# smoggy-P/gym-Drone2D-ActivePerception

Hardware: AMD Instinct MI355X
Metric: env-steps/sec (batched) at 10 agents, map_id=1 (higher is better)
Workload: dtype f64

## Files before the change

gym-drone2d-activeperception_amd/csrc/d2d_hip.hip:

```cpp
#include <hip/hip_runtime.h>
#include <math.h>
#include <stdint.h>
#include <stdio.h>
#include <stdlib.h>
#include <string.h>
#include <type_traits>

#if defined(__HIP_DEVICE_COMPILE__)
#define D2D_AS __attribute__((address_space(1)))
#endif
#include "../../include/d2d.h"
#include "../../include/d2d_hooks.h"
#include "../../include/d2d_stepped.h"
#include "../../include/d2d_swept.h"

#define D2D_TAN_QUAL __device__ __forceinline__
#define D2D_TAN_TBL_QUAL __device__ const
#include "d2d_tan.h"
#define D2D_LOG_QUAL __device__ __forceinline__
#define D2D_LOG_TBL_QUAL __device__ const
#define D2D_RNG_QUAL __device__ __forceinline__
#include "d2d_rng.h"

#define WAVE 64
// ... 647 lines not shown
  }
  return ncand;
}

template <typename M>
struct RayT {
  double xs, ys;
  M cmask;
};
template <typename M>
__device__ __forceinline__ int mask_first(M m) {
  if constexpr (sizeof(M) == 8) return __ffsll((long long)m) - 1;
  else return __ffs((int)m) - 1;
}

template <typename M>
__device__ __forceinline__ RayT<M> ray_setup(const d2d_cfg &c, const LdsView &L, int i, int ncand, double x0, double y0,
                                             double yaw0) {
  const double ss = c.scale - 1.0;
  const double rad90 = 0x1.921fb54442d18p+0, rad270 = 0x1.2d97c7f3321d2p+2;
  const double pi_ = 0x1.921fb54442d18p+1;
  const double player_angle = 0x1.921fb54442d18p+2 - yaw0 * 0x1.1df46a2529d39p-6;
  const double ang = positive_angle(player_angle + (c.ray_off0 + c.ray_dth * (double)i));
  const bool faced_right = (ang < rad90 || ang > rad270);
  const bool faced_up = (ang > pi_);
#ifdef D2D_ABL_NOTAN
  double slope = ang * 0.3;
#else
  double slope = d2d_tan(ang);
#endif
  RayT<M> ry;
  if (fabs(slope) > 1.0) {
    slope = 1.0 / slope;
    ry.ys = faced_up ? -ss : ss;
    ry.xs = ry.ys * slope;
  } else {
    ry.xs = faced_right ? ss : -ss;
    ry.ys = ry.xs * slope;
  }
  ry.cmask = 0;
  if (ncand <= (int)(8 * sizeof(M))) {
    const double len2 = ry.xs * ry.xs + ry.ys * ry.ys, l1 = fabs(ry.xs) + fabs(ry.ys);
    for (int q = 0; q < ncand; ++q) {
      const double ex = L.cx[q] - x0, ey = L.cy[q] - y0, rq = L.crr[q] + 1e-6;
      const double cr = ex * ry.ys - ey * ry.xs, dt = ex * ry.xs + ey * ry.ys;
      const bool near_line = cr * cr <= rq * rq * len2 * (1.0 + 1e-9);
      const bool ahead = dt + rq * l1 >= 0.0;
      ry.cmask |= (near_line && ahead) ? (M)((M)1 << q) : (M)0;
    }
  }
  return ry;
}

template <bool GENERAL, bool FULL, typename M, typename GX>
__device__ __forceinline__ void ray_march(const GX &gx, const d2d_cfg &c, const Geom &g, const LdsView &L, const RayT<M> &ry, bool active,
                                          int ncand, double x0, double y0, const Tile &wt, const Tile &ct, bool patch,
                                          unsigned char *__restrict__ dm) {
  const int H = c.H;
  const CellDiv cell(c.scale, fmax(c.W_px, c.H_px));
  const double depth2 = c.depth * c.depth;
  const bool mask_path = ncand <= (int)(8 * sizeof(M));
  const unsigned char *gtw = (const unsigned char *)L.gtw;
  unsigned char *dmt = (unsigned char *)L.dmt;
  double x = x0 + ry.xs, y = y0 + ry.ys;
  bool alive = active && (0.0 < x && x < c.W_px && 0.0 < y && y < c.H_px);
  const int klo = g.klo;
  const bool has1 = mask_path && ry.cmask != (M)0;
  const int q1 = has1 ? mask_first(ry.cmask) : 0;
  const double c1x = L.cx[q1], c1y = L.cy[q1], c1r2 = has1 ? L.cr2[q1] : -1.0;
  const int c1i = L.cidx[q1];
  const M rest = mask_path ? (M)(ry.cmask & (ry.cmask - (M)1)) : (M)0;
  const bool some1 = __any(has1);
  auto sample = [&](auto far_tag) {
    constexpr bool FAR = decltype(far_tag)::value;
    bool any = false;
    if (some1) {
      const double dx = c1x - x, dy = c1y - y;
      any = alive && (dx * dx + dy * dy <= c1r2);
      if (any) L.hit[c1i] = 1;
    }
    if (GENERAL && mask_path) {
      M m = alive ? rest : (M)0;
      while (m) {
        const int q = mask_first(m);
        m &= m - (M)1;
        const double dx = L.cx[q] - x, dy = L.cy[q] - y;
        if (dx * dx + dy * dy <= L.cr2[q]) {
          L.hit[L.cidx[q]] = 1;
          any = true;
        }
      }
    } else if (GENERAL && alive) {
      if (ncand <= g.ccap) {
        for (int q = 0; q < ncand; ++q) {
          const double dx = L.cx[q] - x, dy = L.cy[q] - y;
          if (dx * dx + dy * dy <= L.cr2[q]) {
            L.hit[L.cidx[q]] = 1;
            any = true;
          }
        }
      } else {
        for (int k = 0; k < c.N; ++k) {
          const double dx = L.ax[k] - x, dy = L.ay[k] - y;
          if (dx * dx + dy * dy <= L.ar2[k]) {
            L.hit[k] = 1;
            any = true;
          }
        }
      }
    }
    const int ci = cell(x), cj = cell(y);
    unsigned int gi = 0;
    unsigned char wall;
    if constexpr (FULL) {
      gi = alive ? (unsigned int)(ci * H + cj) : 0u;
      wall = gtw[gi];
    } else {
      const int wr = min(max(ci - wt.i0, 0), wt.rows - 1), wq = min(max(cj - wt.j0, 0), wt.cols - 1);
      wall = gtw[wt.byte_index(wr, wq)];
    }
    bool far = false;
    if (FAR) far = ((x - x0) * (x - x0) + (y - y0) * (y - y0) >= depth2);
    const bool stop = (wall == D2D_OCCUPIED) || far;
    const bool write = alive && !any && (!stop || wall == D2D_OCCUPIED);
    if (write) {
      const unsigned char v = stop ? (unsigned char)D2D_OCCUPIED : (unsigned char)D2D_UNOCCUPIED;
      if constexpr (FULL) {
        dm[gi] = v;
        if (patch) dmt[gi] = v;
      } else {
        dm[(unsigned int)gx(ci, cj)] = v;
        const unsigned int pr = (unsigned int)(ci - ct.i0), pq = (unsigned int)(cj - ct.j0);
        if (patch && pr < (unsigned int)ct.rows && pq < (unsigned int)ct.cols) dmt[pr * ct.cols + pq] = v;
      }
    }
    alive = alive && !any && !stop;
    x = x + ry.xs;
    y = y + ry.ys;
    alive = alive && (0.0 < x && x < c.W_px && 0.0 < y && y < c.H_px);
  };
#ifndef D2D_ABL_NOMARCH
  const int k1 = min(klo + 1, g.smax);
#pragma unroll 1
  for (int k = 1; k < k1; ++k) sample(std::false_type{});
#pragma unroll 1
  for (int k = max(k1, 1); k < g.smax; ++k) sample(std::true_type{});
#endif
}

struct DynCells {
  unsigned int pclr;
  unsigned int nfree;
};

__device__ __forceinline__ void dyn_bitmap(const d2d_cfg &c, int lane, const Geom &g, const LdsView &L) {
  const int N = c.N, W = c.W, H = c.H;
  if (g.bmw == 0) return;
  for (int w = lane; w < g.bmw; w += WAVE) L.bm[w] = 0u;
  wave_sync_lds();
  for (int k = lane; k < N; k += WAVE) {
    const int cx = L.ncx[k], cy = L.ncy[k], u = L.nu[k];
    const int i1 = min(cx + u + 1, W), j1 = min(cy + u + 1, H);
    for (int i = max(cx - u, 0); i < i1; ++i)
      for (int j = max(cy - u, 0); j < j1; ++j) {
        const int bit = i * H + j;
        atomicOr(&L.bm[bit >> 5], 1u << (bit & 31));
      }
  }
}
// ... 662 lines not shown
    frz = ((double)r.steps >= c.max_steps && !dead) ? 1 : 0;
  }
  const int done = (col != 0) || dead || frz || (r.sm == D2D_SM_GOAL_REACHED && r.tnext >= r.ntgt);
  if (done && c.kf_enabled) {
    int an = 0, ats = 0;
    for (int k = lane; k < N; k += WAVE) {
      if (L.act[k] != 0) {
        an += 1;
        ats += L.klen[k];
      }
    }
    r.bufn += wave_sum(an);
    r.bufts += wave_sum(ats);
  }
  if (lane == 0) {
    unsigned char *f = s.flags + (size_t)e * 4;
    f[D2D_F_COLLISION] = (unsigned char)col;
    f[D2D_F_DEADLOCK] = (unsigned char)dead;
    f[D2D_F_FREEZING] = (unsigned char)frz;
    f[D2D_F_DONE] = (unsigned char)done;
  }
  r.done = done;
}

__device__ __forceinline__ void st_obs(const d2d_cfg &c, const d2d_state &s, int e, int lane, const LdsView &L,
                                       const EnvRegs &r) {
  const int n = c.L * c.L;
  unsigned char *__restrict__ ob = s.obs_local + (size_t)e * n;
  const unsigned char *dmt = (const unsigned char *)L.dmt;
  for (int idx = lane; idx < n; idx += WAVE) ob[idx] = dmt[idx];
  if (lane == 0) s.obs_yaw[e] = (float)r.yaw;
}

__device__ __forceinline__ void load_regs(const d2d_state &s, int e, EnvRegs &r) {
  const double *d = s.drone + (size_t)e * D2D_DF;
  r.x = d[D2D_D_X]; r.y = d[D2D_D_Y]; r.yaw = d[D2D_D_YAW];
  r.vx = d[D2D_D_VX]; r.vy = d[D2D_D_VY]; r.ax = d[D2D_D_AX]; r.ay = d[D2D_D_AY];
  r.tx = s.target[(size_t)e * 2]; r.ty = s.target[(size_t)e * 2 + 1];
  const int *cn = s.counters + (size_t)e * D2D_CF;
  r.steps = cn[D2D_C_STEPS]; r.fail = cn[D2D_C_FAIL]; r.sm = cn[D2D_C_SM]; r.tnext = cn[D2D_C_TGT_NEXT];
  r.ntgt = cn[D2D_C_NTGT]; r.tracked = cn[D2D_C_TRACKED]; r.bufn = cn[D2D_C_BUF_N]; r.bufts = cn[D2D_C_BUF_TS];
}

__device__ __forceinline__ void store_regs(const d2d_state &s, int e, const EnvRegs &r) {
  double *d = s.drone + (size_t)e * D2D_DF;
  d[D2D_D_X] = r.x; d[D2D_D_Y] = r.y; d[D2D_D_YAW] = r.yaw;
  d[D2D_D_VX] = r.vx; d[D2D_D_VY] = r.vy; d[D2D_D_AX] = r.ax; d[D2D_D_AY] = r.ay;
  s.target[(size_t)e * 2] = r.tx; s.target[(size_t)e * 2 + 1] = r.ty;
  int *cn = s.counters + (size_t)e * D2D_CF;
  cn[D2D_C_STEPS] = r.steps; cn[D2D_C_FAIL] = r.fail; cn[D2D_C_SM] = r.sm; cn[D2D_C_TGT_NEXT] = r.tnext;
  cn[D2D_C_TRACKED] = r.tracked; cn[D2D_C_BUF_N] = r.bufn; cn[D2D_C_BUF_TS] = r.bufts;
}

template <bool FULL, bool WIDE, bool CONE, bool TILED = false>
__device__ __forceinline__ void run_env(const d2d_cfg &c, const d2d_state &s, int e, int lane, uint32_t stages,
                                        const Geom &g, const LdsView &L, double action, EnvRegs &r, size_t noise_off = 0,
                                        bool load_r = false, const StepIn *given = nullptr, bool late_obs = false,
                                        int *dyn_gate = nullptr, bool dyn_visible = true, bool dyn_skip = false) {
  using RayMask = std::conditional_t<WIDE, unsigned long long, unsigned int>;
  const int N = c.N, W = c.W, H = c.H;
  const double inv_scale = 1.0 / c.scale;
  const bool do_ray = stages & D2D_ST_RAYCAST, do_dyn = (stages & D2D_ST_DYNGRID) && !dyn_skip, do_trk = stages & D2D_ST_TRACKER;
  const bool do_col = stages & D2D_ST_COLLIDE, do_obs = stages & D2D_ST_OBS, do_ctl = stages & D2D_ST_CONTROL;
  const GridIx<TILED> gx = {H, (H + 15) >> 4};
  const size_t gbytes = TILED ? (size_t)((W + 15) >> 4) * (size_t)((H + 15) >> 4) * 256 : (size_t)W * H;
  unsigned char *__restrict__ gt = s.gt + (size_t)e * gbytes;
  unsigned char *__restrict__ dm = s.dmap + (size_t)e * gbytes;

  const bool gt_staged = FULL && (do_ray || do_dyn);
  const uint32_t needs_agents = D2D_ST_AGENTS | D2D_ST_RAYCAST | D2D_ST_DYNGRID | D2D_ST_TRACKER | D2D_ST_COLLIDE;
  const bool agents_light = (stages & needs_agents) && !(stages & (D2D_ST_AGENTS | D2D_ST_RAYCAST | D2D_ST_DYNGRID));
  StepInRaw in_raw;
  AgentIn ag0;
  const bool agents_any = (stages & needs_agents) != 0;
  if (load_r) {
    in_raw.use = false;
    if (do_ctl && !given) load_inputs_raw(c, s, e, true, in_raw);
    agent_load(c, s, e, lane, do_trk || do_col, ag0, agents_light);
  }
  if constexpr (FULL) {
    if (gt_staged) grid_stage(gt, L.gtw, W * H, lane);
    if (do_obs) grid_stage(dm, L.dmt, W * H, lane);
  }
  if (load_r) {
    if (do_trk && c.kf_enabled && g.kf_lds) kf_stage(c, s, e, lane, L);
    load_regs(s, e, r);
    __builtin_amdgcn_sched_barrier(0);
  }
  StepIn in;
  if (given) {
    in = *given;
    in.action = action;
  } else if (load_r) {
    finish_inputs(in_raw, action, in);
  } else {
    load_inputs(c, s, e, action, do_ctl, in);
  }
  D2D_STAMP(1);
  if (stages & D2D_ST_FSM) st_fsm(c, s, e, r);
  const double x0 = r.x, y0 = r.y, yaw0 = r.yaw;
  if (do_ctl) st_control(c, in, r);
  D2D_STAMP(2);
  if (!load_r && do_trk && c.kf_enabled && g.kf_lds) kf_stage(c, s, e, lane, L);
  if (agents_any) {
    const bool move = (stages & D2D_ST_AGENTS) != 0;
    if (load_r) {
      if (lane < N) agent_apply(c, s, e, lane, L, inv_scale, move, agents_light, ag0);
      if (N > WAVE) st_agents(c, s, e, lane, g, L, inv_scale, move, do_trk || do_col, agents_light, WAVE);
    } else {
      st_agents_plain(c, s, e, lane, g, L, inv_scale, move, do_trk || do_col, agents_light, do_dyn || !dyn_gate);
    }
    if (do_trk && !do_ray)
      for (int k = lane; k < N; k += WAVE) L.hit[k] = s.hit[(size_t)e * N + k];
    wave_sync_lds();
  }
  D2D_STAMP(3);

  const int ocx = cell_fast(x0, c.scale, inv_scale), ocy = cell_fast(y0, c.scale, inv_scale);
  const int ncx_d = cell_fast(r.x, c.scale, inv_scale), ncy_d = cell_fast(r.y, c.scale, inv_scale);
  const int edge = (c.L - 1) / 2;
  const Tile wt = make_tile(ocx - g.reach, ocy - g.reach, g.ws, g.ws);
  const Tile ct = make_tile(ncx_d - edge, ncy_d - edge, c.L, c.L);
  bool probe_wall = false;
  const bool dyn_fast = do_dyn;
  DynCells dc;
  dc.pclr = dc.nfree = 0;
  if (do_col && lane < 5 && !gt_staged) {
    const double R = c.drone_radius;
    const double ox = (lane == 0) ? -R : (lane == 2 ? R : 0.0);
    const double oy = (lane == 3) ? -R : (lane == 4 ? R : 0.0);
    const double qx = r.x + ox, qy = r.y + oy;
    const bool oob = (qx >= c.W_px || qx < 0.0 || qy >= c.H_px || qy < 0.0);
    const int pi = min(max(cell_fast(qx, c.scale, inv_scale), 0), W - 1), pj = min(max(cell_fast(qy, c.scale, inv_scale), 0), H - 1);
    probe_wall = oob || gt[gx(pi, pj)] == D2D_OCCUPIED;
  }
  if constexpr (!FULL) {
    if (do_ray && do_obs && wt.cols <= 32 && wt.rows <= 24 && ct.cols <= 33 && ct.rows <= 34) {
      tile_rows2(gx, wt, (unsigned char *)L.gtw, gt, W, H, lane, (unsigned char)D2D_OCCUPIED,
                 ct, (unsigned char *)L.dmt, dm, (unsigned char)0);
    } else {
      if (do_ray) tile_load<9>(gx, wt, (unsigned char *)L.gtw, gt, W, H, lane, (unsigned char)D2D_OCCUPIED);
      if (do_obs) tile_load<9>(gx, ct, (unsigned char *)L.dmt, dm, W, H, lane, (unsigned char)0);
    }
    if (do_dyn) dyn_bitmap(c, lane, g, L);
    if (dyn_fast && lane < N) {
      if (g.dyn2p) dyn_load<true, false>(gx, c, gt, lane, L, dc);
      else dyn_load(gx, c, gt, lane, L, dc);
    }
  }

  int ncand = 0;
  if (do_ray) {
    ncand = ray_cull<CONE>(c, lane, L, x0, y0, yaw0, g.ccap);
  }
  wave_sync_lds();
  D2D_STAMP(4);
  auto landed = [&]() {
    asm volatile("s_waitcnt vmcnt(0)" ::: "memory");
    wave_sync_lds();
    if constexpr (FULL) {
      if (do_col && lane < 5 && gt_staged) {
        const double R = c.drone_radius;
        const double ox = (lane == 0) ? -R : (lane == 2 ? R : 0.0);
        const double oy = (lane == 3) ? -R : (lane == 4 ? R : 0.0);
        const double qx = r.x + ox, qy = r.y + oy;
        const bool oob = (qx >= c.W_px || qx < 0.0 || qy >= c.H_px || qy < 0.0);
        const int pi = min(max(cell_fast(qx, c.scale, inv_scale), 0), W - 1), pj = min(max(cell_fast(qy, c.scale, inv_scale), 0), H - 1);
        probe_wall = oob || ((const unsigned char *)L.gtw)[pi * H + pj] == D2D_OCCUPIED;
      }
    }
  };
  int newly = 0;
  if (do_ray) {
    bool go = false;
    for (int i0 = 0; i0 < c.R; i0 += WAVE) {
      const int i = i0 + lane;
      const RayT<RayMask> ry = ray_setup<RayMask>(c, L, i, ncand, x0, y0, yaw0);
      if (i0 == 0) {
        landed();
        D2D_STAMP(5);
        go = (0.0 < x0 && x0 < c.W_px && 0.0 < y0 && y0 < c.H_px);
        bool cover = false;
        if (ncand <= g.ccap) {
          for (int q = lane; q < ncand; q += WAVE) {
            const double dx = L.cx[q] - x0, dy = L.cy[q] - y0;
            if (go && dx * dx + dy * dy <= L.cr2[q]) {
              L.hit[L.cidx[q]] = 1;
              cover = true;
            }
          }
        } else {
          for (int k = lane; k < N; k += WAVE) {
            const double dx = L.ax[k] - x0, dy = L.ay[k] - y0;
            if (go && dx * dx + dy * dy <= L.ar2[k]) {
              L.hit[k] = 1;
              cover = true;
            }
          }
        }
        go = go && !__any(cover);
        if (go) {
          const int g0 = FULL ? ocx * H + ocy : wt.byte_index(g.reach, g.reach);
          const unsigned char w0 = ((const unsigned char *)L.gtw)[g0];
          const unsigned char v0 = (w0 == D2D_OCCUPIED) ? (unsigned char)D2D_OCCUPIED : (unsigned char)D2D_UNOCCUPIED;
          if (lane == 0) {
            dm[gx(ocx, ocy)] = v0;
            if constexpr (FULL) {
              if (do_obs) ((unsigned char *)L.dmt)[g0] = v0;
            } else {
              const unsigned int pr = (unsigned int)(ocx - ct.i0), pq = (unsigned int)(ocy - ct.j0);
              if (do_obs && pr < (unsigned int)ct.rows && pq < (unsigned int)ct.cols) ((unsigned char *)L.dmt)[pr * ct.cols + pq] = v0;
            }
          }
          go = (w0 != D2D_OCCUPIED);
        }
      }
      const bool general = ncand > (int)(8 * sizeof(RayMask)) || __any((ry.cmask & (ry.cmask - (RayMask)1)) != (RayMask)0);
      if (general) ray_march<true, FULL>(gx, c, g, L, ry, go && i < c.R, ncand, x0, y0, wt, ct, do_obs, dm);
      else ray_march<false, FULL>(gx, c, g, L, ry, go && i < c.R, ncand, x0, y0, wt, ct, do_obs, dm);
    }
    wave_sync_lds();
    D2D_STAMP(6);
    for (int k0 = 0; k0 < N; k0 += WAVE) {
      const int k = k0 + lane;
      bool nw = false;
      if (k < N) {
        const unsigned char h = L.hit[k];
        s.hit[(size_t)e * N + k] = h;
        nw = h && !L.act[k];
      }
      newly += __popcll(__ballot(nw));
    }
    if (lane == 0) s.newly[e] = newly;
    r.tracked += newly;
  } else if (FULL ? (do_obs || do_trk || do_dyn || do_col) : (do_obs || do_trk)) {
    landed();
  }
  D2D_STAMP(7);
  if (do_trk) {
    const double D2D_AS *nz = s.noise;
    if (c.sigma != 0.0 && !s.noise && s.rng) {
      st_noise_draw(c, s, e, lane, L);
      nz = s.rng_draws;
      noise_off = 0;
    }
    if (FULL && g.ncap <= 16) {
      st_tracker_elem(c, s, e, lane, g, L, r, nz, noise_off);
    } else {
      if (g.kf_lds) st_tracker_quad<true>(c, s, e, lane, g, L, r, nz, noise_off);
      else st_tracker_quad<false>(c, s, e, lane, g, L, r, nz, noise_off);
    }
  }
  D2D_STAMP(8);
  if (do_dyn) {
    if constexpr (FULL) {
      bool run = true;
      if (dyn_gate) {
        int gs = __builtin_amdgcn_readfirstlane(*dyn_gate);
        if (gs == 0) gs = dyn_gate_full(c, lane, L) ? 1 : 2;
        *dyn_gate = gs;
        run = dyn_visible || gs == 2;
      }
      if (run) dyn_full(c, s, e, lane, L, gt);
    } else if (g.dyn2p) {
      if (lane < N) dyn_apply<1>(gx, c, s, e, lane, g, L, gt, dc);
      for (int k = WAVE + lane; k < N; k += WAVE) {
        DynCells dk;
        dyn_load<true, false>(gx, c, gt, k, L, dk);
        dyn_apply<1>(gx, c, s, e, k, g, L, gt, dk);
      }
      wave_sync_global();
      for (int k = lane; k < N; k += WAVE) {
        DynCells dk;
        dyn_load<false, true>(gx, c, gt, k, L, dk);
        dyn_apply<2>(gx, c, s, e, k, g, L, gt, dk);
      }
    } else {
      if (lane < N) dyn_apply<0>(gx, c, s, e, lane, g, L, gt, dc);
      for (int k = WAVE + lane; k < N; k += WAVE) {
        DynCells dk;
        dyn_load(gx, c, gt, k, L, dk);
        dyn_apply<0>(gx, c, s, e, k, g, L, gt, dk);
      }
    }
  }
  D2D_STAMP(9);
  if (do_col) st_collide(c, s, e, lane, L, probe_wall, r);
  D2D_STAMP(10);
  D2D_STAMP(11);
  if (do_obs) {
    wave_sync_lds();
    if constexpr (FULL) obs_full(c, s, e, lane, L, ncx_d, ncy_d, r);
    else st_obs(c, s, e, lane, L, r);
  } else if (late_obs && __builtin_amdgcn_readfirstlane(r.done)) {
    wave_sync_global();
    if constexpr (FULL) grid_stage(dm, L.dmt, W * H, lane);
    else tile_load<9>(gx, ct, (unsigned char *)L.dmt, dm, W, H, lane, (unsigned char)0);
    asm volatile("s_waitcnt vmcnt(0)" ::: "memory");
    wave_sync_lds();
    if constexpr (FULL) obs_full(c, s, e, lane, L, ncx_d, ncy_d, r);
    else st_obs(c, s, e, lane, L, r);
  }
  D2D_STAMP(12);
}

#include "d2d_plan_spec.h"
__host__ __device__ constexpr bool spec_full(int spec) { return spec == 1 || spec == 2; }
__host__ __device__ constexpr bool spec_wide(int spec) { return spec == 3 || spec == 0 || spec == 4; }
__host__ __device__ constexpr bool spec_tiled(int spec) { return spec == 4; }
__host__ __device__ constexpr bool spec_generic(int spec) { return spec == 0 || spec == 4; }
__host__ __device__ constexpr bool spec_cone(int spec) { return spec != 1; }
extern __shared__ __attribute__((aligned(16))) char d2d_lds[];
// ... 95 lines not shown
  }
}

__global__ __launch_bounds__(WAVE *WAVES_PER_BLOCK) void k_reset(d2d_cfg c, d2d_state s, d2d_state init,
                                                                 const unsigned char *mask, int mask_stride) {
  const int lane = threadIdx.x & (WAVE - 1), wv = threadIdx.x / WAVE;
  const int e = blockIdx.x * WAVES_PER_BLOCK + wv;
  if (e >= c.B) return;
  if (mask && !mask[(size_t)e * mask_stride]) return;
  reset_env(c, s, init, (size_t)e, lane);
}

__global__ void k_tan(const double *in, double *out, long long n) {
  const long long i = (long long)blockIdx.x * blockDim.x + threadIdx.x;
  if (i < n) out[i] = d2d_tan(in[i]);
}

__global__ void k_log(const double *x, double *out, long long n) {
  const long long i = (long long)blockIdx.x * blockDim.x + threadIdx.x;
  if (i < n) out[i] = d2d_log(x[i]);
}

__global__ __launch_bounds__(WAVE) void k_rng_draw(uint32_t *rng, const int *m, double *out, int max_m) {
  const int lane = threadIdx.x;
  uint32_t *st = rng + (size_t)blockIdx.x * D2D_RNG_WORDS;
  double *o = out + (size_t)blockIdx.x * max_m * 2;
  const int mb = __builtin_amdgcn_readfirstlane(min(max(m[blockIdx.x], 0), max_m));
  int pos = __builtin_amdgcn_readfirstlane((int)st[D2D_RNG_POS]);
  const bool bad = !rng_pos_ok(pos);
  int got = 0, regen = 0;
  if (!bad)
    got = rng_wave_pairs(st, pos, regen, d2d_rng_regen_cap(mb), mb, lane, [&](int q, double v0, double v1) {
      o[(size_t)q * 2] = v0;
      o[(size_t)q * 2 + 1] = v1;
    });
  for (int k = got + lane; k < max_m; k += WAVE) o[(size_t)k * 2] = o[(size_t)k * 2 + 1] = k < mb ? __builtin_nan("") : 0.0;
  if (!bad) rng_wave_store(st, pos, got, regen, lane);
}

#include "d2d_plugins.h"

__global__ void k_atan2(const double *y, const double *x, double *out, long long n) {
  const long long i = (long long)blockIdx.x * blockDim.x + threadIdx.x;
  if (i < n) out[i] = d2d_atan2(y[i], x[i]);
}

struct ClosedArgs {
  d2d_cfg c;
  d2d_state s;
  d2d_plan p;
  d2d_state init;
  int on_done, nsteps;
  int obs_every;
};
static_assert(sizeof(ClosedArgs) <= D2D_LAUNCH_ARGS_BYTES, "d2d_plan.launch_args (D2D_LAUNCH_ARGS_BYTES) is too small for the parked launch arguments");

__global__ void k_closed_args(ClosedArgs *dst, d2d_cfg c, d2d_state s, d2d_plan p, d2d_state init, int on_done, int nsteps, int obs_every) {
  if (threadIdx.x == 0 && blockIdx.x == 0) {
    dst->c = c;
    dst->s = s;
    dst->p = p;
    dst->init = init;
    dst->on_done = on_done;
    dst->nsteps = nsteps;
    dst->obs_every = obs_every;
  }
}

template <int SPEC>
__host__ __device__ inline int closed_wave_bytes(const d2d_cfg &c, const d2d_plan &p, int wpb) {
  int b = make_geom(c, wpb, spec_ncap(SPEC), spec_full(SPEC)).wave_bytes;
  const int pb = plan_wave_bytes(c.N, p.nu, p.n_sample, c.W, c.H), gb = p.gaze == D2D_GAZE_OXFORD ? gaze_geom(c, p).wave_bytes : 0;
  b = b > pb ? b : pb;
  b = b > gb ? b : gb;
  return (b + 15) & ~15;
}


#if defined(__HIP_DEVICE_COMPILE__)
typedef const ClosedArgs __attribute__((address_space(4))) *ArgsPtr;
#else
typedef const ClosedArgs *ArgsPtr;
#endif

struct PhaseIn {
  ArgsPtr a;
  int e, off, lane;
};
__device__ __forceinline__ PhaseIn phase_enter(const ClosedArgs *ap, int e_, int lds_off_) {
  const unsigned long long v = (unsigned long long)ap;
  unsigned int lo = __builtin_amdgcn_readfirstlane((unsigned int)v), hi = __builtin_amdgcn_readfirstlane((unsigned int)(v >> 32));
  int e = __builtin_amdgcn_readfirstlane(e_), off = __builtin_amdgcn_readfirstlane(lds_off_);
  int lane = threadIdx.x & (WAVE - 1);
  asm volatile("; phase" : "+s"(lo), "+s"(hi), "+s"(e), "+s"(off), "+v"(lane));
  PhaseIn in;
  in.a = (ArgsPtr)(((unsigned long long)hi << 32) | lo);
  in.e = e;
  in.off = off;
  in.lane = lane;
  return in;
}
template <bool PDEF, typename F>
__device__ __forceinline__ auto with_plan(ArgsPtr a, F f) {
  if constexpr (PDEF) {
    d2d_plan p = a->p;
    plan_default_apply(p);
    return f(p);
  } else {
    return f(a->p);
  }
}


template <int SPEC, bool PDEF>
__device__ __forceinline__ int ph_plan_quick(const ClosedArgs *ap, int e_, int lds_off_) {
  const PhaseIn in_ = phase_enter(ap, e_, lds_off_);
  const ArgsPtr a = in_.a;
  const int e = in_.e, lane = in_.lane;
// ... 17 lines not shown
  char *base = d2d_lds + in_.off;
  d2d_cfg c = a->c;
  if (!spec_generic(SPEC)) spec_default_apply(c);
  if constexpr (SPEC == 1 || SPEC == 2) {
    constexpr int cap = spec_ncap(SPEC);
    __builtin_assume(c.N <= cap);
  }
  with_plan<PDEF>(a, [&](const d2d_plan &p) __attribute__((always_inline)) { plan_env_search<PDEF>(c, a->s, p, e, lane, base); });
  wave_sync_global();
}

__host__ __device__ constexpr uint32_t hidden_stages(uint32_t stages) { return stages & ~(uint32_t)D2D_ST_OBS; }
__host__ __device__ constexpr bool late_obs_of(uint32_t stages) { return (stages & D2D_ST_COLLIDE) && !(stages & D2D_ST_OBS); }


template <int SPEC, bool PDEF, uint32_t ACT = D2D_ST_ACT>
__device__ __forceinline__ int ph_plan_act(const ClosedArgs *ap, int e_, int lds_off_, int &walls_ok) {
  const PhaseIn in_ = phase_enter(ap, e_, lds_off_);
  const ArgsPtr a = in_.a;
  const int e = in_.e, lane = in_.lane;
  char *base = d2d_lds + in_.off;
  d2d_cfg c = a->c;
  if (!spec_generic(SPEC)) spec_default_apply(c);
  if constexpr (SPEC == 1 || SPEC == 2) {
    constexpr int cap = spec_ncap(SPEC);
    __builtin_assume(c.N <= cap);
  }
  double4 w_head;
  int wk = __builtin_amdgcn_readfirstlane(walls_ok);
  asm volatile("; phase" : "+s"(wk));
  const bool need = with_plan<PDEF>(a, [&](const d2d_plan &p) __attribute__((always_inline)) { return plan_env_quick(c, a->s, p, e, lane, base, &w_head, &wk); });
  walls_ok = __builtin_amdgcn_readfirstlane(wk);
  if (need) {
    wave_sync_global();
    return -1;
  }
  wave_sync_lds();
  StepIn in;
  in.action = 0.0;
  in.ok = true;
  in.has_wp = true;
  in.wp[0] = w_head.x; in.wp[1] = w_head.y; in.wp[2] = w_head.z; in.wp[3] = w_head.w; in.wp[4] = 0.0; in.wp[5] = 0.0;
  const int wpb = (int)(blockDim.x / WAVE);
  const Geom g = make_geom(c, wpb, spec_ncap(SPEC), spec_full(SPEC));
  const LdsView L = carve(base, g, c.L);
  EnvRegs r;
  run_env<spec_full(SPEC), spec_wide(SPEC), spec_cone(SPEC), spec_tiled(SPEC)>(c, a->s, e, lane, ACT, g, L, a->s.action[e], r, 0, true, &in, late_obs_of(ACT));
  if (lane == 0) store_regs(a->s, e, r);
  wave_sync_global();
  return r.done;
}

template <int SPEC, bool PDEF, uint32_t STAGES>
__device__ __forceinline__ int ph_gaze_stages(const ClosedArgs *ap, int e_, int lds_off_, int t_, int done_, int &dyn_gate, bool dyn_vis_) {
  const PhaseIn in_ = phase_enter(ap, e_, lds_off_);
  const ArgsPtr a = in_.a;
  const int e = in_.e, lane = in_.lane;
  int tstep = __builtin_amdgcn_readfirstlane(t_), known_done = __builtin_amdgcn_readfirstlane(done_);
  asm volatile("; phase" : "+s"(tstep), "+s"(known_done));
  int dgate = 2;
  const int dvis = dyn_vis_ ? 1 : 0;
  if constexpr (spec_full(SPEC)) {
    dgate = __builtin_amdgcn_readfirstlane(dyn_gate);
    asm volatile("; phase" : "+s"(dgate));
  }
  char *base = d2d_lds + in_.off;
  d2d_cfg c = a->c;
  if (!spec_generic(SPEC)) spec_default_apply(c);
#ifdef D2D_CHAIN_PROF
  const unsigned long long pp0 = __builtin_amdgcn_s_memtime();
#endif
  with_plan<PDEF>(a, [&](const d2d_plan &p) __attribute__((always_inline)) {
    gaze_env<true, PDEF>(c, a->s, p, a->init, a->on_done == D2D_DONE_RESET, e, lane, base, known_done);
  });
  wave_sync_global();
#ifdef D2D_CHAIN_PROF
  D2D_PHASE_ADD(0, pp0);
  const unsigned long long pp1 = __builtin_amdgcn_s_memtime();
#endif
  const int wpb = (int)(blockDim.x / WAVE);
  const Geom g = make_geom(c, wpb, spec_ncap(SPEC), spec_full(SPEC));
  const LdsView L = carve(base, g, c.L);
  EnvRegs r;
  load_regs(a->s, e, r);
  const size_t noise_off = c.noise_rows > 1 ? (size_t)((c.noise_row0 + tstep) % c.noise_rows) * c.B * c.N * 2 : 0;
  if constexpr (spec_full(SPEC)) {
    run_env<true, spec_wide(SPEC), spec_cone(SPEC), spec_tiled(SPEC)>(c, a->s, e, lane, STAGES, g, L, a->s.action[e], r, noise_off, false, nullptr, late_obs_of(STAGES), &dgate, dvis != 0, dgate == 1 && dvis == 0);
    dyn_gate = __builtin_amdgcn_readfirstlane(dgate);
  } else {
    run_env<spec_full(SPEC), spec_wide(SPEC), spec_cone(SPEC), spec_tiled(SPEC)>(c, a->s, e, lane, STAGES, g, L, a->s.action[e], r, noise_off, false, nullptr, late_obs_of(STAGES));
  }
  if (lane == 0) store_regs(a->s, e, r);
  wave_sync_global();
#ifdef D2D_CHAIN_PROF
  D2D_PHASE_ADD(1, pp1);
#endif
  return r.done;
}

template <int SPEC, uint32_t STAGES>
__device__ __forceinline__ int ph_stages(const ClosedArgs *ap, int e_, int lds_off_) {
  const PhaseIn in_ = phase_enter(ap, e_, lds_off_);
  const ArgsPtr a = in_.a;
  const int e = in_.e, lane = in_.lane;
  char *base = d2d_lds + in_.off;
  d2d_cfg c = a->c;
  if (!spec_generic(SPEC)) spec_default_apply(c);
  const int wpb = (int)(blockDim.x / WAVE);
  const Geom g = make_geom(c, wpb, spec_ncap(SPEC), spec_full(SPEC));
  const LdsView L = carve(base, g, c.L);
  EnvRegs r;
  run_env<spec_full(SPEC), spec_wide(SPEC), spec_cone(SPEC), spec_tiled(SPEC)>(c, a->s, e, lane, STAGES, g, L, a->s.action[e], r, 0, true, nullptr, late_obs_of(STAGES));
  if (lane == 0) store_regs(a->s, e, r);
  wave_sync_global();
  return r.done;
}

template <int SPEC, bool PDEF = false>
__global__ __launch_bounds__(WAVE *WAVES_PER_BLOCK, D2D_MIN_WAVES) void k_closed(const ClosedArgs *__restrict__ a) {
  static_assert(!PDEF || SPEC == 1, "the plan's defaults are folded into the few-agent kernel of the default geometry only");
  const int wv = __builtin_amdgcn_readfirstlane(threadIdx.x / WAVE);
  const int wpb = (int)(blockDim.x / WAVE);
  const int e = blockIdx.x * wpb + wv;
  if (e >= a->c.B) return;
  d2d_cfg c = a->c;
  if (!spec_generic(SPEC)) spec_default_apply(c);
  int off;
  bool split;
  if constexpr (PDEF) {
    d2d_plan p = a->p;
    plan_default_apply(p);
    off = wv * closed_wave_bytes<SPEC>(c, p, wpb);
    split = p.planner == D2D_PLAN_PRIMITIVE;
  } else {
    off = wv * closed_wave_bytes<SPEC>(c, a->p, wpb);
    split = a->p.planner == D2D_PLAN_PRIMITIVE;
  }
  const int nsteps = a->nsteps;
  const bool freeze = a->on_done == D2D_DONE_FREEZE;
  const bool obs_every = a->obs_every != 0;
  const bool dyn_defer = spec_full(SPEC) && !obs_every && !freeze, auto_reset = a->on_done == D2D_DONE_RESET;
  int dyn_gate = dyn_defer ? 0 : 2;
  int nsearch = 0;
  int walls_ok = 0;
#ifdef D2D_CHAIN_PROF
  const unsigned long long cp0 = __builtin_amdgcn_s_memtime();
  unsigned long long cps = 0;
#endif
  int flag_done = a->s.flags[(size_t)e * 4 + D2D_F_DONE] != 0 ? 1 : 0;
#pragma unroll 1
  for (int t = 0; t < nsteps; ++t) {
    if (freeze && flag_done != 0) break;
    const bool visible = obs_every || t == nsteps - 1;
    if (dyn_defer && auto_reset && flag_done != 0) dyn_gate = 0;
    if (split) {
      if (nsearch * 32 > t + 16) __builtin_amdgcn_s_setprio(2); else __builtin_amdgcn_s_setprio(0);
      ph_gaze_stages<SPEC, PDEF, D2D_ST_PERCEIVE>(a, e, off, t, flag_done, dyn_gate, visible);
#ifdef D2D_CHAIN_PROF
      const unsigned long long q0 = __builtin_amdgcn_s_memtime();
#endif
      const int pa = __builtin_amdgcn_readfirstlane(visible ? ph_plan_act<SPEC, PDEF, D2D_ST_ACT>(a, e, off, walls_ok)
                                                            : ph_plan_act<SPEC, PDEF, hidden_stages(D2D_ST_ACT)>(a, e, off, walls_ok));
#ifdef D2D_CHAIN_PROF
      D2D_PHASE_ADD(2, q0);
#endif
      if (pa < 0) {
#ifdef D2D_CHAIN_PROF
        const unsigned long long s0 = __builtin_amdgcn_s_memtime();
#endif
        ph_plan_search<SPEC, PDEF>(a, e, off);
        nsearch += 1;
        walls_ok = 0;
#ifdef D2D_CHAIN_PROF
        cps += __builtin_amdgcn_s_memtime() - s0;
        D2D_PHASE_ADD(3, s0);
        const unsigned long long a0 = __builtin_amdgcn_s_memtime();
#endif
        flag_done = __builtin_amdgcn_readfirstlane(visible ? ph_stages<SPEC, D2D_ST_ACT>(a, e, off)
                                                           : ph_stages<SPEC, hidden_stages(D2D_ST_ACT)>(a, e, off));
#ifdef D2D_CHAIN_PROF
        D2D_PHASE_ADD(4, a0);
#endif
      } else {
        flag_done = pa;
      }
    } else {
      flag_done = __builtin_amdgcn_readfirstlane(visible ? ph_gaze_stages<SPEC, PDEF, D2D_ST_ALL>(a, e, off, t, flag_done, dyn_gate, true)
                                                         : ph_gaze_stages<SPEC, PDEF, hidden_stages(D2D_ST_ALL)>(a, e, off, t, flag_done, dyn_gate, false));
    }
  }
#ifdef D2D_CHAIN_PROF
  if ((threadIdx.x & (WAVE - 1)) == 0 && a->p.plan_stat) {
    const unsigned long long tot = __builtin_amdgcn_s_memtime() - cp0;
    a->p.plan_stat[(size_t)e * 4 + 1] = (int)(tot >> 4);
    a->p.plan_stat[(size_t)e * 4 + 2] = (int)(cps >> 4);
  }
#endif
}

#include "d2d_swept.h"

thread_local char g_err[256] = "";

int fail(int code, const char *msg) {
  snprintf(g_err, sizeof g_err, "%s", msg);
  return code;
}

constexpr size_t LDS_SOFT = 64 * 1024, LDS_HARD = 160 * 1024;

template <typename K>
void lds_optin(K kernel, size_t bytes) {
  if (bytes > LDS_SOFT) (void)hipFuncSetAttribute((const void *)kernel, hipFuncAttributeMaxDynamicSharedMemorySize, (int)bytes);
}

int launched() {
  const hipError_t err = hipGetLastError();
  return err == hipSuccess ? 0 : fail(-3, hipGetErrorString(err));
}

dim3 env_grid(int B, int wpb = WAVES_PER_BLOCK) { return dim3((B + wpb - 1) / wpb); }
dim3 env_block(int wpb = WAVES_PER_BLOCK) { return dim3(WAVE * wpb); }

int spec_of(const d2d_cfg &c) {
  if (!spec_default_matches(c)) return c.grid_tile ? 4 : 0;
  return c.N <= spec_ncap(1) ? 1 : (c.N <= spec_ncap(2) ? 2 : 3);
}

[[maybe_unused]] const void *const kInstantiationOrder[] = {
    (const void *)k_stages<3>, (const void *)k_stages<1>, (const void *)k_stages<2>, (const void *)k_stages<4>, (const void *)k_stages<0>,
    (const void *)k_closed<0>, (const void *)k_closed<4>, (const void *)k_closed<3>, (const void *)k_closed<1>, (const void *)k_closed<2>,
    (const void *)k_closed<1, true>};

template <typename F>
auto with_spec(int spec, F f) {
  switch (spec) {
    case 1: return f(IntC<1>{});
    case 2: return f(IntC<2>{});
    case 3: return f(IntC<3>{});
    case 4: return f(IntC<4>{});
    default: return f(IntC<0>{});
// ... 268 lines not shown

int d2d_reset(const d2d_cfg *c, const d2d_state *s, const d2d_state *init, const uint8_t *mask, void *stream) {
  return reset_launch(c, s, init, mask, 1, stream);
}

int d2d_gaze_stage(const d2d_cfg *c, const d2d_state *s, const d2d_plan *p, void *stream) {
  int rc = plan_check(c, s, p);
  if (rc) return rc;
  return gaze_launch(c, s, p, nullptr, false, stream);
}

int d2d_plan_stage(const d2d_cfg *c, const d2d_state *s, const d2d_plan *p, void *stream) {
  int rc = plan_check(c, s, p);
  if (rc) return rc;
  return plan_launch(c, s, p, false, stream);
}

int d2d_gaze_stage_live(const d2d_cfg *c, const d2d_state *s, const d2d_plan *p, void *stream) {
  int rc = plan_check(c, s, p);
  if (rc) return rc;
  return gaze_launch(c, s, p, nullptr, true, stream);
}

int d2d_plan_stage_live(const d2d_cfg *c, const d2d_state *s, const d2d_plan *p, void *stream) {
  int rc = plan_check(c, s, p);
  if (rc) return rc;
  return plan_launch(c, s, p, true, stream);
}

#define D2D_SWEPT_ENTRY_POINTS
#include "d2d_swept.h"

int d2d_plan_reset(const d2d_cfg *c, const d2d_plan *p, const uint8_t *mask, int32_t mask_stride, void *stream) {
  if (!c || !p) return fail(-1, "null cfg/plan");
  if (c->abi_version != D2D_ABI_VERSION) return fail(-2, "ABI version mismatch");
  return plan_reset_launch(c, p, mask, mask_stride, stream);
}

int d2d_closed_loop(const d2d_cfg *c, const d2d_state *s, const d2d_plan *p, int32_t nsteps, int32_t on_done,
                    const d2d_state *init, void *stream) {
  int rc = plan_check(c, s, p);
  if (rc) return rc;
  if (nsteps < 0) return fail(-1, "closed_loop: bad step count");
  if (on_done < D2D_DONE_CONTINUE || on_done > D2D_DONE_FREEZE) return fail(-1, "closed_loop: bad on_done");
  const bool auto_reset = on_done == D2D_DONE_RESET;
  if (auto_reset && !snapshot_complete(init)) return fail(-1, "closed_loop: D2D_DONE_RESET needs the snapshot");
  if (c->B == 0 || nsteps == 0) return 0;
  if (c->planner_mode == D2D_PLANNER_EXTERNAL && p->launch_args && (p->planner == D2D_PLAN_PRIMITIVE || p->gaze != D2D_GAZE_NONE)) {
    const Launch l = pick_launch(*c, p);
    if (l.wpb >= 1) {
      ClosedArgs *dev = (ClosedArgs *)p->launch_args;
      const char *obs_env = getenv("D2D_OBS_EVERY_STEP");
      const bool obs_every = obs_env && obs_env[0] == '1' && obs_env[1] == '\0';
      hipLaunchKernelGGL(k_closed_args, dim3(1), dim3(64), 0, (hipStream_t)stream, dev, *c, *s, *p, auto_reset ? *init : *s,
                         (int)on_done, (int)nsteps, obs_every ? 1 : 0);
      auto launch = [&](auto kernel) {
        lds_optin(kernel, l.lds());
        hipLaunchKernelGGL(kernel, env_grid(c->B, l.wpb), env_block(l.wpb), l.lds(), (hipStream_t)stream, (const ClosedArgs *)dev);
      };
      const char *fold_env = getenv("D2D_PLAN_FOLD");
      const bool fold_off = fold_env && fold_env[0] == '0' && fold_env[1] == '\0';
      if (l.spec == 1 && !fold_off && plan_default_matches(*c, *p)) launch(k_closed<1, true>);
      else with_spec(l.spec, [&](auto S) { launch(k_closed<decltype(S)::value>); });
      return launched();
    }
  }
  const bool split = p->planner == D2D_PLAN_PRIMITIVE;
  const uint32_t skip = on_done == D2D_DONE_FREEZE ? D2D_ST_SKIP_DONE : 0;
  for (int32_t t = 0; t < nsteps; ++t) {
    if ((rc = gaze_launch(c, s, p, auto_reset ? init : nullptr, skip != 0, stream))) return rc;
    d2d_state sn = *s;
    sn.noise = noise_row(c, s, t);
    if (split) {
      if ((rc = launch_stages(c, &sn, D2D_ST_PERCEIVE | skip, stream))) return rc;
      if ((rc = plan_launch(c, s, p, skip != 0, stream))) return rc;
      if ((rc = launch_stages(c, s, D2D_ST_ACT | skip, stream))) return rc;
    } else if ((rc = launch_stages(c, &sn, D2D_ST_ALL | skip, stream))) {
      return rc;
    }
  }
  return 0;
}

int d2d_launch_shape(const d2d_cfg *c, const d2d_plan *p, int32_t out[4]) {
  if (!c || !out) return fail(-1, "launch_shape: null argument");
  if (c->abi_version != D2D_ABI_VERSION) return fail(-2, "ABI version mismatch");
  Launch l = pick_launch(*c, p);
  if (p && (!p->launch_args || c->planner_mode != D2D_PLANNER_EXTERNAL)) l.wpb = 0;
  out[0] = l.wpb;
  out[1] = (int32_t)l.lds();
  out[2] = out[1] > 0 ? (int32_t)(LDS_HARD / (size_t)out[1]) : 0;
  out[3] = spec_full(l.spec) ? 1 : 0;
  return 0;
}

int d2d_sincos_array(const double *in, double *so, double *co, int64_t n, void *stream) {
  return launch_array(k_sincos, n, n > 0 && (!in || !so || !co), "sincos_array: bad arguments", stream, in, so, co);
}

int d2d_tan_array(const double *in, double *out, int64_t n, void *stream) {
  return launch_array(k_tan, n, n > 0 && (!in || !out), "tan_array: bad arguments", stream, in, out);
}

int d2d_atan2_array(const double *y, const double *x, double *out, int64_t n, void *stream) {
  return launch_array(k_atan2, n, n > 0 && (!y || !x || !out), "atan2_array: bad arguments", stream, y, x, out);
}

int d2d_log_array(const double *x, double *out, int64_t n, void *stream) {
// ... 16 lines not shown
```

Measured before the change: 104.3 million.

## Cache ground-truth grid as per-lane wall bitmasks in registers

When the dynamic grid gate marks an env as static, each lane packs one column of the ground-truth occupancy grid into a 64-bit wall bitmask held in registers across steps. Later steps then write these compact bitmasks to LDS instead of re-staging the full byte grid from global memory. Ray marching and probe wall checks read single bits instead of bytes. This is meant to cut global loads and LDS traffic per step, at the cost of extra VGPRs and the assumption that H fits in 64 bits and W fits within one lane per column.

```diff
diff --git a/gym-drone2d-activeperception_amd/csrc/d2d_hip.hip b/gym-drone2d-activeperception_amd/csrc/d2d_hip.hip
--- a/gym-drone2d-activeperception_amd/csrc/d2d_hip.hip
+++ b/gym-drone2d-activeperception_amd/csrc/d2d_hip.hip
@@ -723,7 +723,42 @@
   return ry;
 }
 
-template <bool GENERAL, bool FULL, typename M, typename GX>
+struct GtRows {
+  unsigned int lo, hi;
+  int on;
+};
+__device__ __forceinline__ void gt_rows_build(const d2d_cfg &c, int lane, const LdsView &L, GtRows &rw) {
+  const int H = c.H, last = (c.W * H - 1) >> 2, ndw = (H + 3) >> 2;
+  const int b0 = min(lane, c.W - 1) * H, a = b0 >> 2;
+  const unsigned int sh = (unsigned int)(b0 & 3);
+  unsigned int lo = 0, hi = 0;
+  unsigned int prev = L.gtw[a];
+#pragma unroll
+  for (int k = 0; k < ndw; ++k) {
+    const unsigned int next = L.gtw[min(a + k + 1, last)];
+    const unsigned int w = __builtin_amdgcn_alignbyte(next, prev, sh);
+    prev = next;
+    const unsigned int x = w ^ (0x01010101u * D2D_OCCUPIED);
+    const unsigned int z = ~(((x & 0x7f7f7f7fu) + 0x7f7f7f7fu) | x | 0x7f7f7f7fu);
+    unsigned int nib = (((z >> 7) * 0x00204081u) >> 21) & 0xfu;
+    if (H - 4 * k < 4) nib &= (1u << (H - 4 * k)) - 1u;
+    if (4 * k < 32) lo |= nib << (4 * k);
+    else hi |= nib << (4 * k - 32);
+  }
+  rw.lo = lo;
+  rw.hi = hi;
+}
+__device__ __forceinline__ void gt_rows_put(const d2d_cfg &c, int lane, const LdsView &L, const GtRows &rw) {
+  if (lane < c.W) {
+    L.gtw[2 * lane] = rw.lo;
+    L.gtw[2 * lane + 1] = rw.hi;
+  }
+}
+__device__ __forceinline__ bool gt_rows_bit(const LdsView &L, int ci, int cj) {
+  return (L.gtw[2 * ci + ((cj >> 5) & 1)] >> (cj & 31)) & 1u;
+}
+
+template <bool GENERAL, bool FULL, bool ROWS, typename M, typename GX>
 __device__ __forceinline__ void ray_march(const GX &gx, const d2d_cfg &c, const Geom &g, const LdsView &L, const RayT<M> &ry, bool active,
                                           int ncand, double x0, double y0, const Tile &wt, const Tile &ct, bool patch,
                                           unsigned char *__restrict__ dm) {
@@ -785,7 +820,8 @@
     unsigned char wall;
     if constexpr (FULL) {
       gi = alive ? (unsigned int)(ci * H + cj) : 0u;
-      wall = gtw[gi];
+      if constexpr (ROWS) wall = gt_rows_bit(L, alive ? ci : 0, cj) ? D2D_OCCUPIED : D2D_UNOCCUPIED;
+      else wall = gtw[gi];
     } else {
       const int wr = min(max(ci - wt.i0, 0), wt.rows - 1), wq = min(max(cj - wt.j0, 0), wt.cols - 1);
       wall = gtw[wt.byte_index(wr, wq)];
@@ -1554,11 +1590,12 @@
   cn[D2D_C_TRACKED] = r.tracked; cn[D2D_C_BUF_N] = r.bufn; cn[D2D_C_BUF_TS] = r.bufts;
 }
 
-template <bool FULL, bool WIDE, bool CONE, bool TILED = false>
+template <bool FULL, bool WIDE, bool CONE, bool TILED = false, bool GTROWS = false>
 __device__ __forceinline__ void run_env(const d2d_cfg &c, const d2d_state &s, int e, int lane, uint32_t stages,
                                         const Geom &g, const LdsView &L, double action, EnvRegs &r, size_t noise_off = 0,
                                         bool load_r = false, const StepIn *given = nullptr, bool late_obs = false,
-                                        int *dyn_gate = nullptr, bool dyn_visible = true, bool dyn_skip = false) {
+                                        int *dyn_gate = nullptr, bool dyn_visible = true, bool dyn_skip = false,
+                                        GtRows *rows = nullptr) {
   using RayMask = std::conditional_t<WIDE, unsigned long long, unsigned int>;
   const int N = c.N, W = c.W, H = c.H;
   const double inv_scale = 1.0 / c.scale;
@@ -1570,6 +1607,8 @@
   unsigned char *__restrict__ dm = s.dmap + (size_t)e * gbytes;
 
   const bool gt_staged = FULL && (do_ray || do_dyn);
+  bool gt_rows = false;
+  if constexpr (FULL && GTROWS) gt_rows = dyn_skip && rows->on != 0;
   const uint32_t needs_agents = D2D_ST_AGENTS | D2D_ST_RAYCAST | D2D_ST_DYNGRID | D2D_ST_TRACKER | D2D_ST_COLLIDE;
   const bool agents_light = (stages & needs_agents) && !(stages & (D2D_ST_AGENTS | D2D_ST_RAYCAST | D2D_ST_DYNGRID));
   StepInRaw in_raw;
@@ -1581,7 +1620,12 @@
     agent_load(c, s, e, lane, do_trk || do_col, ag0, agents_light);
   }
   if constexpr (FULL) {
-    if (gt_staged) grid_stage(gt, L.gtw, W * H, lane);
+    if constexpr (GTROWS) {
+      if (gt_rows) gt_rows_put(c, lane, L, *rows);
+      else if (gt_staged) grid_stage(gt, L.gtw, W * H, lane);
+    } else {
+      if (gt_staged) grid_stage(gt, L.gtw, W * H, lane);
+    }
     if (do_obs) grid_stage(dm, L.dmt, W * H, lane);
   }
   if (load_r) {
@@ -1668,7 +1712,12 @@
         const double qx = r.x + ox, qy = r.y + oy;
         const bool oob = (qx >= c.W_px || qx < 0.0 || qy >= c.H_px || qy < 0.0);
         const int pi = min(max(cell_fast(qx, c.scale, inv_scale), 0), W - 1), pj = min(max(cell_fast(qy, c.scale, inv_scale), 0), H - 1);
-        probe_wall = oob || ((const unsigned char *)L.gtw)[pi * H + pj] == D2D_OCCUPIED;
+        if constexpr (GTROWS) {
+          if (gt_rows) probe_wall = oob || gt_rows_bit(L, pi, pj);
+          else probe_wall = oob || ((const unsigned char *)L.gtw)[pi * H + pj] == D2D_OCCUPIED;
+        } else {
+          probe_wall = oob || ((const unsigned char *)L.gtw)[pi * H + pj] == D2D_OCCUPIED;
+        }
       }
     }
   };
@@ -1703,7 +1752,9 @@
         go = go && !__any(cover);
         if (go) {
           const int g0 = FULL ? ocx * H + ocy : wt.byte_index(g.reach, g.reach);
-          const unsigned char w0 = ((const unsigned char *)L.gtw)[g0];
+          unsigned char w0;
+          if (FULL && GTROWS && gt_rows) w0 = gt_rows_bit(L, ocx, ocy) ? D2D_OCCUPIED : D2D_UNOCCUPIED;
+          else w0 = ((const unsigned char *)L.gtw)[g0];
           const unsigned char v0 = (w0 == D2D_OCCUPIED) ? (unsigned char)D2D_OCCUPIED : (unsigned char)D2D_UNOCCUPIED;
           if (lane == 0) {
             dm[gx(ocx, ocy)] = v0;
@@ -1718,8 +1769,11 @@
         }
       }
       const bool general = ncand > (int)(8 * sizeof(RayMask)) || __any((ry.cmask & (ry.cmask - (RayMask)1)) != (RayMask)0);
-      if (general) ray_march<true, FULL>(gx, c, g, L, ry, go && i < c.R, ncand, x0, y0, wt, ct, do_obs, dm);
-      else ray_march<false, FULL>(gx, c, g, L, ry, go && i < c.R, ncand, x0, y0, wt, ct, do_obs, dm);
+      if (FULL && GTROWS && gt_rows) {
+        if (general) ray_march<true, FULL, FULL && GTROWS>(gx, c, g, L, ry, go && i < c.R, ncand, x0, y0, wt, ct, do_obs, dm);
+        else ray_march<false, FULL, FULL && GTROWS>(gx, c, g, L, ry, go && i < c.R, ncand, x0, y0, wt, ct, do_obs, dm);
+      } else if (general) ray_march<true, FULL, false>(gx, c, g, L, ry, go && i < c.R, ncand, x0, y0, wt, ct, do_obs, dm);
+      else ray_march<false, FULL, false>(gx, c, g, L, ry, go && i < c.R, ncand, x0, y0, wt, ct, do_obs, dm);
     }
     wave_sync_lds();
     D2D_STAMP(6);
@@ -1759,7 +1813,10 @@
       bool run = true;
       if (dyn_gate) {
         int gs = __builtin_amdgcn_readfirstlane(*dyn_gate);
-        if (gs == 0) gs = dyn_gate_full(c, lane, L) ? 1 : 2;
+        if (gs == 0) {
+          gs = dyn_gate_full(c, lane, L) ? 1 : 2;
+          if (GTROWS && gs == 1 && rows->on != 0) gt_rows_build(c, lane, L, *rows);
+        }
         *dyn_gate = gs;
         run = dyn_visible || gs == 2;
       }
@@ -1961,10 +2018,12 @@
   d2d_state init;
   int on_done, nsteps;
   int obs_every;
+  int gt_rows;
 };
 static_assert(sizeof(ClosedArgs) <= D2D_LAUNCH_ARGS_BYTES, "d2d_plan.launch_args (D2D_LAUNCH_ARGS_BYTES) is too small for the parked launch arguments");
 
-__global__ void k_closed_args(ClosedArgs *dst, d2d_cfg c, d2d_state s, d2d_plan p, d2d_state init, int on_done, int nsteps, int obs_every) {
+__global__ void k_closed_args(ClosedArgs *dst, d2d_cfg c, d2d_state s, d2d_plan p, d2d_state init, int on_done, int nsteps, int obs_every,
+                              int gt_rows) {
   if (threadIdx.x == 0 && blockIdx.x == 0) {
     dst->c = c;
     dst->s = s;
@@ -1973,6 +2032,7 @@
     dst->on_done = on_done;
     dst->nsteps = nsteps;
     dst->obs_every = obs_every;
+    dst->gt_rows = gt_rows;
   }
 }
 
@@ -2096,7 +2156,8 @@
 }
 
 template <int SPEC, bool PDEF, uint32_t STAGES>
-__device__ __forceinline__ int ph_gaze_stages(const ClosedArgs *ap, int e_, int lds_off_, int t_, int done_, int &dyn_gate, bool dyn_vis_) {
+__device__ __forceinline__ int ph_gaze_stages(const ClosedArgs *ap, int e_, int lds_off_, int t_, int done_, int &dyn_gate, bool dyn_vis_,
+                                              unsigned int &rows_lo, unsigned int &rows_hi) {
   const PhaseIn in_ = phase_enter(ap, e_, lds_off_);
   const ArgsPtr a = in_.a;
   const int e = in_.e, lane = in_.lane;
@@ -2104,9 +2165,12 @@
   asm volatile("; phase" : "+s"(tstep), "+s"(known_done));
   int dgate = 2;
   const int dvis = dyn_vis_ ? 1 : 0;
+  GtRows rw;
   if constexpr (spec_full(SPEC)) {
     dgate = __builtin_amdgcn_readfirstlane(dyn_gate);
-    asm volatile("; phase" : "+s"(dgate));
+    rw.lo = rows_lo;
+    rw.hi = rows_hi;
+    asm volatile("; phase" : "+s"(dgate), "+v"(rw.lo), "+v"(rw.hi));
   }
   char *base = d2d_lds + in_.off;
   d2d_cfg c = a->c;
@@ -2127,10 +2191,13 @@
   const LdsView L = carve(base, g, c.L);
   EnvRegs r;
   load_regs(a->s, e, r);
+  if constexpr (spec_full(SPEC)) rw.on = a->gt_rows;
   const size_t noise_off = c.noise_rows > 1 ? (size_t)((c.noise_row0 + tstep) % c.noise_rows) * c.B * c.N * 2 : 0;
   if constexpr (spec_full(SPEC)) {
-    run_env<true, spec_wide(SPEC), spec_cone(SPEC), spec_tiled(SPEC)>(c, a->s, e, lane, STAGES, g, L, a->s.action[e], r, noise_off, false, nullptr, late_obs_of(STAGES), &dgate, dvis != 0, dgate == 1 && dvis == 0);
+    run_env<true, spec_wide(SPEC), spec_cone(SPEC), spec_tiled(SPEC), true>(c, a->s, e, lane, STAGES, g, L, a->s.action[e], r, noise_off, false, nullptr, late_obs_of(STAGES), &dgate, dvis != 0, dgate == 1 && dvis == 0, &rw);
     dyn_gate = __builtin_amdgcn_readfirstlane(dgate);
+    rows_lo = rw.lo;
+    rows_hi = rw.hi;
   } else {
     run_env<spec_full(SPEC), spec_wide(SPEC), spec_cone(SPEC), spec_tiled(SPEC)>(c, a->s, e, lane, STAGES, g, L, a->s.action[e], r, noise_off, false, nullptr, late_obs_of(STAGES));
   }
@@ -2185,6 +2252,7 @@
   const bool obs_every = a->obs_every != 0;
   const bool dyn_defer = spec_full(SPEC) && !obs_every && !freeze, auto_reset = a->on_done == D2D_DONE_RESET;
   int dyn_gate = dyn_defer ? 0 : 2;
+  unsigned int rows_lo = 0, rows_hi = 0;
   int nsearch = 0;
   int walls_ok = 0;
 #ifdef D2D_CHAIN_PROF
@@ -2199,7 +2267,7 @@
     if (dyn_defer && auto_reset && flag_done != 0) dyn_gate = 0;
     if (split) {
       if (nsearch * 32 > t + 16) __builtin_amdgcn_s_setprio(2); else __builtin_amdgcn_s_setprio(0);
-      ph_gaze_stages<SPEC, PDEF, D2D_ST_PERCEIVE>(a, e, off, t, flag_done, dyn_gate, visible);
+      ph_gaze_stages<SPEC, PDEF, D2D_ST_PERCEIVE>(a, e, off, t, flag_done, dyn_gate, visible, rows_lo, rows_hi);
 #ifdef D2D_CHAIN_PROF
       const unsigned long long q0 = __builtin_amdgcn_s_memtime();
 #endif
@@ -2229,8 +2297,8 @@
         flag_done = pa;
       }
     } else {
-      flag_done = __builtin_amdgcn_readfirstlane(visible ? ph_gaze_stages<SPEC, PDEF, D2D_ST_ALL>(a, e, off, t, flag_done, dyn_gate, true)
-                                                         : ph_gaze_stages<SPEC, PDEF, hidden_stages(D2D_ST_ALL)>(a, e, off, t, flag_done, dyn_gate, false));
+      flag_done = __builtin_amdgcn_readfirstlane(visible ? ph_gaze_stages<SPEC, PDEF, D2D_ST_ALL>(a, e, off, t, flag_done, dyn_gate, true, rows_lo, rows_hi)
+                                                         : ph_gaze_stages<SPEC, PDEF, hidden_stages(D2D_ST_ALL)>(a, e, off, t, flag_done, dyn_gate, false, rows_lo, rows_hi));
     }
   }
 #ifdef D2D_CHAIN_PROF
@@ -2605,8 +2673,10 @@
       ClosedArgs *dev = (ClosedArgs *)p->launch_args;
       const char *obs_env = getenv("D2D_OBS_EVERY_STEP");
       const bool obs_every = obs_env && obs_env[0] == '1' && obs_env[1] == '\0';
+      const char *rows_env = getenv("D2D_GT_ROWS");
+      const bool rows_off = rows_env && rows_env[0] == '0' && rows_env[1] == '\0';
       hipLaunchKernelGGL(k_closed_args, dim3(1), dim3(64), 0, (hipStream_t)stream, dev, *c, *s, *p, auto_reset ? *init : *s,
-                         (int)on_done, (int)nsteps, obs_every ? 1 : 0);
+                         (int)on_done, (int)nsteps, obs_every ? 1 : 0, rows_off ? 0 : 1);
       auto launch = [&](auto kernel) {
         lds_optin(kernel, l.lds());
         hipLaunchKernelGGL(kernel, env_grid(c->B, l.wpb), env_block(l.wpb), l.lds(), (hipStream_t)stream, (const ClosedArgs *)dev);
```

Measured after the change: 105.2 million (median of 6 runs). Within noise of the previous version (+0.9%).
